# ashispati/ar-vae

Measured on AMD Instinct MI355X. Metric: training images/sec (dSprites beta-VAE+AR, per-GPU batch 512), higher is better.
Workload: dtype f32 (conv MFMAs: scaled 2-term fp16 split, 3 products, fp32-accurate)

## Files before the change

### ar-vae_amd/csrc/common.h

```cpp
#pragma once
#include <hip/hip_runtime.h>
#include <stdint.h>
#include <stdio.h>

#include "../../include/arvae_hip.h"

namespace arvae {

extern thread_local char g_last_error[512];

int fail(int code, const char *fmt, ...);
int check_launch(const char *what);
void prof_gap();
bool profiling_active();

#define ARVAE_LAUNCH(...)                  \
    do {                                   \
        ::arvae::prof_gap();               \
        hipLaunchKernelGGL(__VA_ARGS__);   \
    } while (0)

#define ARVAE_REQUIRE(cond, ...)                                   \
    do {                                                           \
        if (!(cond)) return ::arvae::fail(ARVAE_E_INVALID, __VA_ARGS__); \
    } while (0)

static inline int sample_filter_check(const char *who, const arvae_sample_filter_t *filter, int32_t vocab, int *k_eff, bool *active) {
    ARVAE_REQUIRE(filter != nullptr, "%s: null filter", who);
    ARVAE_REQUIRE(filter->top_k >= 0 && filter->top_k <= vocab, "%s: top_k %d is outside [0, %d] (0 = off)", who, filter->top_k, vocab);
    ARVAE_REQUIRE(filter->top_p > 0.f && filter->top_p <= 1.f, "%s: top_p %f is not in (0, 1] (1 = off)", who,
                  (double)filter->top_p);
    *k_eff = filter->top_k == 0 ? vocab : filter->top_k;
    *active = *k_eff < vocab || filter->top_p < 1.f || filter->allow != nullptr;
    return ARVAE_OK;
}

static inline int note_plan_check(const char *who, const arvae_note_plan_t *plan, int64_t ticks, int32_t vocab) {
    ARVAE_REQUIRE(plan != nullptr, "%s: null plan", who);
    ARVAE_REQUIRE(plan->allow != nullptr, "%s: null plan mask (plan->allow)", who);
    ARVAE_REQUIRE(ticks >= 1 && vocab >= 1, "%s: a plan of %lld ticks and %d notes", who, (long long)ticks, vocab);
// ... 193 lines not shown
```

### ar-vae_amd/csrc/conv32.hip

```cpp
#include "diag.h"
#include "launch.h"
#include "conv32_common.h"
#include "conv32.h"
#include "reduce.h"
#include "midprep.h"
#include "prep32.h"
#include "regloss.h"
#include "down32p.h"
#include "wgrad32r.h"
#include "stamps.h"

#include <type_traits>

namespace arvae {

template <int LO, int STRIDE, int PX = 128>
struct PatchLoader {
    using T = Tile<LO, PX>;
    static constexpr int SZ = STRIDE * LO;
    static constexpr int PR = STRIDE * T::TR + 2, PC = STRIDE * T::TC + 2;
    static constexpr int SLOTS = T::TI * PR * PC * 8;
    static constexpr int ITERS = (SLOTS + 255) / 256;
    float4 r[ITERS];
    unsigned rel[ITERS];
// ... 71 lines not shown
                uint2 hv, lv;
                split2(r[it].x, r[it].y, sc, hv.x, lv.x);
                split2(r[it].z, r[it].w, sc, hv.y, lv.y);
                unsigned *d = buf + pix * PSB2 + q * 2;
                *reinterpret_cast<uint2 *>(d) = hv;
                *reinterpret_cast<uint2 *>(d + 16) = lv;
            }
        }
    }
};

#ifdef ARVAE_STAMPS_CONV32
ARVAE_STAMP_TABLE(conv32, 512, 64, 2)
#define STAMP(slot) do { if (LO == 16 && threadIdx.x == 0) ARVAE_STAMP(g_conv32_stamps, BID, slot); } while (0)
#define STAMP_WAIT() stamp_wait_all()
#define PSTAMP(role, slot) do { if (threadIdx.x == 256 * (role) && BID < 256) ARVAE_STAMP(g_conv32_stamps, BID + 256 * (role), slot); } while (0)
#else
#define STAMP(slot)
#define STAMP_WAIT()
#define PSTAMP(role, slot)
#endif


template <int MODE>
__device__ __forceinline__ unsigned store_group(const f32x16 &acc, int g, float inv, const float4 &b, const float4 &gv, unsigned gbits,
                                                __amdgpu_buffer_rsrc_t rs_out, unsigned off, bool live, float &amax) {
    float v[4] = {fmaf(acc[4 * g], inv, b.x), fmaf(acc[4 * g + 1], inv, b.y), fmaf(acc[4 * g + 2], inv, b.z), fmaf(acc[4 * g + 3], inv, b.w)};
    const float gf[4] = {gv.x, gv.y, gv.z, gv.w};
    unsigned bits = 0;
#pragma unroll
    for (int j = 0; j < 4; ++j) {
        if (MODE == EP_RELU) {
            v[j] = fmaxf(v[j], 0.f);
            bits |= (v[j] > 0.f ? 1u : 0u) << (4 * g + j);
        }
        if (MODE == EP_GATE_F) v[j] = gf[j] > 0.f ? v[j] : 0.f;
        if (MODE == EP_GATE_B) v[j] = ((gbits >> (4 * g + j)) & 1u) ? v[j] : 0.f;
    }
    const float4 o = make_float4(v[0], v[1], v[2], v[3]);
    amax = live ? fmaxf(amax, amax4(o)) : amax;
    buf_store4(o, rs_out, off + g * 32);
    return bits;
}

template <int MODE>
__device__ __forceinline__ void store_pixel(const f32x16 &acc, float inv, const float4 (&b4)[4], __amdgpu_buffer_rsrc_t rs_out,
                                            __amdgpu_buffer_rsrc_t rs_gate, __amdgpu_buffer_rsrc_t rs_bits, bool want_bits,
                                            unsigned off, int half, bool live, float &amax) {
    float4 gv[4];
    unsigned gb = 0;
#pragma unroll
    for (int g = 0; g < 4; ++g) gv[g] = make_float4(0.f, 0.f, 0.f, 0.f);
    if (MODE == EP_GATE_F) {
#pragma unroll
        for (int g = 0; g < 4; ++g) gv[g] = buf_load4(rs_gate, off + g * 32);
    }
    if (MODE == EP_GATE_B) gb = buf_load_u16(rs_bits, bits_off(off, half));
    unsigned bits = 0;
#pragma unroll
    for (int g = 0; g < 4; ++g) bits |= store_group<MODE>(acc, g, inv, b4[g], gv[g], gb, rs_out, off, live, amax);
    if (MODE == EP_RELU && want_bits) buf_store_u16(bits, rs_bits, bits_off(off, half));
}

__device__ __forceinline__ void load_bias4(const float *bias, int half, float4 (&b4)[4]) {
#pragma unroll
    for (int g = 0; g < 4; ++g)
        b4[g] = bias != nullptr ? *reinterpret_cast<const float4 *>(bias + 8 * g + 4 * half) : make_float4(0.f, 0.f, 0.f, 0.f);
}

__global__ __launch_bounds__(256) void conv32_weight_prep_kernel(PrepArgs p) { conv32_prep_block(p, blockIdx.x); }

__global__ __launch_bounds__(256) void prep_all_kernel(PrepArgs p, MidPrepArgs mid, int conv_blocks) {
    prep_all_block(p, mid, conv_blocks, blockIdx.x);
}

__global__ __launch_bounds__(256) void amax_kernel(const float *__restrict__ x, int64_t count4, unsigned *__restrict__ out) {
    __shared__ float wm[4];
    float m = 0.f;
    const int64_t stride = (int64_t)gridDim.x * 256;
    for (int64_t i = (int64_t)blockIdx.x * 256 + threadIdx.x; i < count4; i += 4 * stride) {
        float4 v[4];
#pragma unroll
        for (int u = 0; u < 4; ++u) {
// ... 64 lines not shown
            tile_origin<LO, PX>(tile + NBLK, ni, nr);
            pl.set_tile(ni, nr, tile + NBLK < n_tiles);
            pl.issue_all();
        }
        f32x16 acc;
#pragma unroll
        for (int i = 0; i < 16; ++i) acc[i] = 0.f;
#pragma unroll
        for (int kx = 0; kx < 4; ++kx)
#pragma unroll
            for (int cc = 0; cc < 2; ++cc) {
                const f16x8 ah = lds_x8<f16x8>(ldsw + aoff + kx * PSB2 + cc * 8), al = lds_x8<f16x8>(ldsw + aoff + kx * PSB2 + cc * 8 + 16);
                MFMA_H(acc, w2[kx][cc][1], ah);
                MFMA_H(acc, w2[kx][cc][0], al);
                MFMA_H(acc, w2[kx][cc][0], ah);
            }
#pragma unroll
        for (int reg = 0; reg < 16; ++reg) red[(wave * 16 + reg) * 64 + lane] = acc[reg];
        __syncthreads();
        if (wave == 0) {
#pragma unroll
            for (int reg = 0; reg < 16; ++reg)
                acc[reg] = (acc[reg] + red[(16 + reg) * 64 + lane]) + (red[(32 + reg) * 64 + lane] + red[(48 + reg) * 64 + lane]);
            store_pixel<MODE>(acc, inv, b4, rs_out, rs_gate, rs_bits, want_bits,
                              out_lane + (unsigned)(((img0 * LO + r0) * LO) * PIXB), half, true, amax_run);
        }
    }
    if (wave == 0) amax_publish(ep.amax_out, BID, NBLK, amax_run);
}
template <int LO, int MODE>
__global__ __launch_bounds__(256, 2) void down32s_kernel(const float *__restrict__ hi, Ep32 ep, int n_img, int n_tiles) {
    down32s_body<LO, MODE>(hi, ep, n_img, n_tiles, blockIdx.x, gridDim.x);
}



constexpr int UP_ISSUE_STEPS = 4;
template <int LO, int MODE, int PX = 128>
__device__ __forceinline__ void up32x_body(const float *__restrict__ lo, Ep32 ep, int n_img, int n_tiles, const int BID, const int NBLK) {
    using PL = PatchLoader<LO, 1, PX>;
    constexpr int MT = PX / 32;
    constexpr int HI = 2 * LO, PC = PL::PC, PR = PL::PR, PLANE = PL::PLANE_DW;
    extern __shared__ __attribute__((aligned(16))) float lds[];
    unsigned *ldsw = reinterpret_cast<unsigned *>(lds);
    const int lane = threadIdx.x & 63, wave = __builtin_amdgcn_readfirstlane(threadIdx.x >> 6);
    const int half = lane >> 5, rc = lane & 31;
    const int py = wave >> 1, px = wave & 1;
// ... 79 lines not shown
#pragma unroll
        for (int mt = 0; mt < MT; ++mt)
#pragma unroll
            for (int i = 0; i < 16; ++i) acc[mt][i] = 0.f;
        f16x8 a[2][MT][2];
#pragma unroll
        for (int mt = 0; mt < MT; ++mt)
#pragma unroll
            for (int t = 0; t < 2; ++t) a[0][mt][t] = lds_x8<f16x8>(ldsw + t * PLANE + aoff[mt]);
        static_for<0, 8>([&](auto sc_) __attribute__((always_inline)) {
            constexpr int step = decltype(sc_)::value, ty = step >> 2, tx = (step >> 1) & 1, c = step & 1;
            constexpr int cur = step & 1, nxt = cur ^ 1;
            constexpr int nstep = step + 1, nty = nstep >> 2, ntx = (nstep >> 1) & 1, nc = nstep & 1;
            constexpr int ntoff = -(nty * PC + ntx) * PSB + nc * 8;
            if constexpr (step < UP_ISSUE_STEPS) pl.template issue_step<UP_ISSUE_STEPS, step>();
            __builtin_amdgcn_sched_barrier(0);
            static_for<0, MT>([&](auto mc) __attribute__((always_inline)) {
                constexpr int sub = decltype(mc)::value;
                constexpr int slot = step * MT + sub;
                if constexpr ((slot & 1) == 0) {
                    constexpr int k = slot >> 1, em = k >> 2, eg = k & 3;
                    const unsigned poff = prev_base + orel[em];
                    if (eg == 0) pbits[em] = 0;
                    pbits[em] |= store_group<MODE>(prev[em], eg, inv, b4[eg], gq[k], gqb[em], rs_out, poff, prev_base != OOB, amax_run);
                    if (MODE == EP_RELU && eg == 3)
                        buf_store_u16(pbits[em], rs_bits, (prev_base == OOB || !want_bits) ? OOB : bits_off(poff, half));
                    if (MODE == EP_GATE_F) gq[k] = buf_load4(rs_gate, obase + orel[em] + eg * 32);
                    if constexpr (MODE == EP_GATE_B && k < MT) gqn[k] = buf_load_u16(rs_bits, bits_off(obase + orel[k], half));
                }
                static_for<3 * sub, 3 * sub + 3>([&](auto qc) __attribute__((always_inline)) {
                    constexpr int m = decltype(qc)::value, prod = m / MT, pm = m % MT;
                    constexpr int tw = prod == 0 ? 1 : 0, ta = prod == 1 ? 1 : 0;
                    MFMA_H(acc[pm], w2[ty][tx][c][tw], a[cur][pm][ta]);
                });
                if constexpr (nstep < 8) {
                    static_for<2 * sub, 2 * sub + 2>([&](auto rc_) __attribute__((always_inline)) {
                        constexpr int ri = decltype(rc_)::value, rmt = ri / 2, rt = ri % 2;
                        a[nxt][rmt][rt] = lds_x8<f16x8>(ldsw + rt * PLANE + aoff[rmt] + ntoff);
                    });
                }
                (void)nxt;
            });
            __builtin_amdgcn_sched_barrier(0);
        });
        STAMP(7 + 6 * stamp_t);
#pragma unroll
        for (int mt = 0; mt < MT; ++mt) prev[mt] = acc[mt];
        if (MODE == EP_GATE_B) {
#pragma unroll
            for (int mt = 0; mt < MT; ++mt) gqb[mt] = gqn[mt];
        }
        prev_base = obase;
        __syncthreads();
        pl.commit_split2(ldsw, sc.s);
        __syncthreads();
        STAMP(8 + 6 * stamp_t);
        ++stamp_t;
    }
#pragma unroll
    for (int mt = 0; mt < MT; ++mt) {
        const unsigned poff = prev_base + orel[mt];
        unsigned bits = 0;
#pragma unroll
        for (int g = 0; g < 4; ++g) bits |= store_group<MODE>(prev[mt], g, inv, b4[g], gq[mt * 4 + g], gqb[mt], rs_out, poff, prev_base != OOB, amax_run);
        if (MODE == EP_RELU) buf_store_u16(bits, rs_bits, (prev_base == OOB || !want_bits) ? OOB : bits_off(poff, half));
    }
    amax_publish(ep.amax_out, BID * 4 + wave, NBLK * 4, amax_run);
    STAMP_WAIT();
    STAMP(63);
}
template <int LO, int MODE, int PX = 128>
__global__ __launch_bounds__(256, 1) void up32x_kernel(const float *__restrict__ lo, Ep32 ep, int n_img, int n_tiles) {
    up32x_body<LO, MODE, PX>(lo, ep, n_img, n_tiles, blockIdx.x, gridDim.x);
}

struct C1Wgrad {
    const float *img;
    float *slab;
};
constexpr int C1W_VP = 16, C1W_XP = 16;
constexpr int C1W_WAVE_DW = 2 * 32 * C1W_VP + 2 * 32 * C1W_XP;
constexpr float C1W_SX = 1024.f, C1W_SX_INV = 1.f / 1024.f;

template <int MODE, bool C1W = false>
__device__ __forceinline__ void up32p_body(const float *__restrict__ lo, Ep32 ep, int n_img, int n_tiles, const int BID, const int NBLK,
                                           C1Wgrad c1 = C1Wgrad{nullptr, nullptr}) {
    static_assert(MODE != EP_GATE_F, "up32p_kernel: float gates stay on up32x_kernel");
    static_assert(!C1W || MODE == EP_GATE_B, "the fused first-layer weight gradient takes the sign-bit gated data gradient");
    constexpr int LO = 16, PX = 128, HI = 2 * LO, MT = PX / 32;
    using PL = PatchLoader<LO, 1, PX>;
    constexpr int PR = PL::PR, PC = PL::PC, PLANE = PL::PLANE_DW, SLOTS = PL::SLOTS, ITERS = PL::ITERS;
    constexpr int BUF = 2 * PLANE;
    extern __shared__ __attribute__((aligned(16))) float lds_f[];
    unsigned *lds = reinterpret_cast<unsigned *>(lds_f);
    float4 *hand = reinterpret_cast<float4 *>(lds + 2 * BUF);
    const int lane = threadIdx.x & 63, wave = __builtin_amdgcn_readfirstlane(threadIdx.x >> 6);
    const int half = lane >> 5, rc = lane & 31;
    const int per_wg = (n_tiles + NBLK - 1) / NBLK, t_first = BID * per_wg;
    const int t_end = min(n_tiles, t_first + per_wg);
    const int cls = wave & 3, py = cls >> 1, px = cls & 1;

    if (wave >= 4) {
        PSTAMP(1, 0);
        int pst = 0;
        (void)pst;
        const AmaxLoad al = amax_issue(ep.amax_in);
        unsigned orel[MT];
#pragma unroll
        for (int mt = 0; mt < MT; ++mt) {
            int img, r, c;
            tile_pixel<LO, PX>(mt * 32 + rc, img, r, c);
            orel[mt] = (unsigned)(((img * HI + 2 * r + py) * HI + 2 * c + px) * PIXB + half * 16);
        }
        const int64_t out_bytes = (int64_t)n_img * HI * HI * PIXB;
        const __amdgpu_buffer_rsrc_t rs_out = make_rsrc(ep.out, out_bytes);
        const bool want_bits = MODE == EP_RELU && ep.bits_out != nullptr;
        const __amdgpu_buffer_rsrc_t rs_bits =
            make_rsrc(MODE == EP_GATE_B ? (const void *)ep.gate_bits : want_bits ? (const void *)ep.bits_out : (const void *)ep.out,
                      (int64_t)n_img * HI * HI * 4);
        float4 b4[4];
        load_bias4(ep.bias, half, b4);
        const float inv = amax_scale(al).inv * prep_inv_scale(ep.wprep);
        float amax_run = 0.f;
        auto tile_base = [&](int tile) -> unsigned {
            int img0, r0;
            tile_origin<LO, PX>(tile, img0, r0);
            return tile < t_end ? (unsigned)(((img0 * HI + 2 * r0) * HI) * PIXB) : OOB;
        };
        unsigned gb[MT] = {}, gbn[MT] = {};
        auto request_gates = [&](unsigned base) __attribute__((always_inline)) {
            if (MODE == EP_GATE_B) {
#pragma unroll
                for (int mt = 0; mt < MT; ++mt) gbn[mt] = buf_load_u16(rs_bits, base == OOB ? OOB : bits_off(base + orel[mt], half));
            }
        };
        auto epilogue = [&](unsigned base) __attribute__((always_inline)) {
            const float4 no_gate = make_float4(0.f, 0.f, 0.f, 0.f);
#pragma unroll
            for (int mt = 0; mt < MT; ++mt) {
                f32x16 acc;
#pragma unroll
                for (int g = 0; g < 4; ++g) {
                    const float4 v = hand[((cls * MT + mt) * 4 + g) * 64 + lane];
                    acc[4 * g] = v.x; acc[4 * g + 1] = v.y; acc[4 * g + 2] = v.z; acc[4 * g + 3] = v.w;
                }
                const unsigned poff = base + orel[mt];
                unsigned bits = 0;
#pragma unroll
                for (int g = 0; g < 4; ++g) bits |= store_group<MODE>(acc, g, inv, b4[g], no_gate, gb[mt], rs_out, poff, base != OOB, amax_run);
                if (MODE == EP_RELU) buf_store_u16(bits, rs_bits, (base == OOB || !want_bits) ? OOB : bits_off(poff, half));
            }
        };
        unsigned *c1_v = lds + 2 * BUF + 4 * MT * 4 * 64 * 4 + (wave - 4) * C1W_WAVE_DW;
        unsigned *c1_x = c1_v + 2 * 32 * C1W_VP;
        f32x16 c1_acc, c1_acc2;
#pragma unroll
        for (int i = 0; i < 16; ++i) { c1_acc[i] = 0.f; c1_acc2[i] = 0.f; }
        const __amdgpu_buffer_rsrc_t rs_img = make_rsrc(C1W ? c1.img : ep.out, C1W ? (int64_t)n_img * 4 * HI * HI * 4 : 0);
        int c1_voff[2][2], c1_xoff[2][2];
        const int c1_sw = 2 * ((rc >> 2) & 7);
        {
            const int g16 = lane >> 4, q = (lane & 15) >> 2, pp = lane & 3;
#pragma unroll
            for (int b = 0; b < 2; ++b)
#pragma unroll
                for (int i = 0; i < 2; ++i) {
                    const int P = 16 * b + 8 * (g16 >> 1) + 4 * i + q;
                    const int sw = 2 * ((P >> 2) & 7);
                    c1_voff[b][i] = P * C1W_VP + ((8 * (g16 & 1) + 2 * pp) ^ sw);
                    c1_xoff[b][i] = P * C1W_XP + ((8 * (g16 & 1) + 2 * pp) ^ sw);
                }
            if constexpr (C1W) {
                const int csw = 2 * ((rc >> 2) & 7);
#pragma unroll
                for (int d = 0; d < 4; ++d) {
                    const int col = 8 + 4 * half + d;
// ... 7 lines not shown
            if constexpr (C1W) {
                int img0, r0;
                tile_origin<LO, PX>(tile, img0, r0);
#pragma unroll
                for (int mt = 0; mt < MT; ++mt) {
                    int im, r, c;
                    tile_pixel<LO, PX>(mt * 32 + rc, im, r, c);
                    const int Y = 2 * (r0 + r) + py, X = 2 * c + px;
#pragma unroll
                    for (int e = 0; e < 2; ++e) {
                        const int iy = 2 * Y - 1 + 2 * half + e, ix = X == 0 ? 0 : 2 * X - 1;
                        const bool ok = tile < t_end && (unsigned)iy < (unsigned)(2 * HI);
                        c1_tapn[mt][e] = buf_load4(rs_img, ok ? (unsigned)((((img0 + im) * 2 * HI + iy) * 2 * HI + ix) * 4) : OOB);
                    }
                }
            }
        };
        auto c1_tile = [&](unsigned base) __attribute__((always_inline)) {
            if constexpr (C1W) {
#pragma unroll
                for (int mt = 0; mt < MT; ++mt) {
#pragma unroll
                    for (int g = 0; g < 4; ++g) {
                        const float4 a = hand[((cls * MT + mt) * 4 + g) * 64 + lane];
                        const unsigned bits = base != OOB ? gb[mt] >> (4 * g) : 0u;
                        const float v0 = (bits & 1u) ? a.x : 0.f, v1 = (bits & 2u) ? a.y : 0.f, v2 = (bits & 4u) ? a.z : 0.f, v3 = (bits & 8u) ? a.w : 0.f;
                        uint2 hv, lv;
                        split2(v0, v1, 0x1p-23f, hv.x, lv.x);
                        split2(v2, v3, 0x1p-23f, hv.y, lv.y);
                        const int vd = (4 * g + 2 * half) ^ c1_sw;
                        *reinterpret_cast<uint2 *>(c1_v + rc * C1W_VP + vd) = hv;
                        *reinterpret_cast<uint2 *>(c1_v + 32 * C1W_VP + rc * C1W_VP + vd) = lv;
                    }
                    {
                        int im, r, c;
                        tile_pixel<LO, PX>(mt * 32 + rc, im, r, c);
                        const int X = 2 * c + px;
                        uint4 hx, lx;
                        unsigned *hp = &hx.x, *lp = &lx.x;
#pragma unroll
                        for (int e = 0; e < 2; ++e) {
                            float4 t = c1_tap[mt][e];
                            if (X == 0) t = make_float4(0.f, t.x, t.y, t.z);
                            if (X == HI - 1) t.w = 0.f;
                            split2(t.x, t.y, C1W_SX, hp[2 * e], lp[2 * e]);
                            split2(t.z, t.w, C1W_SX, hp[2 * e + 1], lp[2 * e + 1]);
                        }
// ... 169 lines not shown
                    constexpr int m = decltype(qc)::value, prod = m / MT, pm = m % MT;
                    constexpr int tw = prod == 0 ? 1 : 0, ta = prod == 1 ? 1 : 0;
                    MFMA_H(acc[pm], w2[ty][tx][c][tw], a[cu][pm][ta]);
                });
                if constexpr (nstep < 8) {
                    static_for<2 * sub, 2 * sub + 2>([&](auto rc_) __attribute__((always_inline)) {
                        constexpr int ri = decltype(rc_)::value, rmt = ri / 2, rt = ri % 2;
                        a[nxt][rmt][rt] = lds_x8<f16x8>(ldsw + rt * PLANE + aoff[rmt] + ntoff);
                    });
                }
                (void)nxt;
                __builtin_amdgcn_sched_barrier(0);
            });
        });
        PSTAMP(0, 4 + 6 * cst);
        commit_tile(lds + (cur ^ 1) * BUF);
        PSTAMP(0, 5 + 6 * cst);
        __syncthreads();
        PSTAMP(0, 6 + 6 * cst);
#pragma unroll
        for (int mt = 0; mt < MT; ++mt)
#pragma unroll
            for (int g = 0; g < 4; ++g)
                hand[((wave * MT + mt) * 4 + g) * 64 + lane] = make_float4(acc[mt][4 * g], acc[mt][4 * g + 1], acc[mt][4 * g + 2], acc[mt][4 * g + 3]);
        PSTAMP(0, 7 + 6 * cst);
        __syncthreads();
        PSTAMP(0, 8 + 6 * cst);
        ++cst;
    }
    PSTAMP(0, 63);
    if constexpr (C1W) {
        __syncthreads();
        __syncthreads();
    }
}
template <int MODE>
__global__ __launch_bounds__(512) __attribute__((amdgpu_waves_per_eu(2, 2))) void up32p_kernel(const float *__restrict__ lo, Ep32 ep,
                                                                                               int n_img, int n_tiles) {
    up32p_body<MODE>(lo, ep, n_img, n_tiles, blockIdx.x, gridDim.x);
}

template <int LO, int MODE>
__global__ __launch_bounds__(256, 1) void up32x_reg_kernel(const float *__restrict__ lo, Ep32 ep, int n_img,
                                                            int n_tiles, int grid_up, RegArgs reg, int reg_bx) {
    if ((int)blockIdx.x < grid_up) {
        up32x_body<LO, MODE, 32>(lo, ep, n_img, n_tiles, blockIdx.x, grid_up);
        return;
// ... 82 lines not shown
            set_lo(ni, nr, tile + NBLK < n_tiles);
        }
        static_for<0, KB>([&](auto bc) __attribute__((always_inline)) {
            constexpr int b = decltype(bc)::value;
            f16x8 b2[2];
#pragma unroll
            for (int t = 0; t < 2; ++t) b2[t] = lds_tr_x8<f16x8>(lo_w + t * LPLANE + loff[b][0], lo_w + t * LPLANE + loff[b][1]);
            pl.template issue_step<KB, b>();
            if constexpr (b < 2) lr[b] = buf_load4(rs_lo, lo_base + b * 4096);
#pragma unroll
            for (int kx = 0; kx < 4; ++kx) {
                f16x8 a2[2];
#pragma unroll
                for (int t = 0; t < 2; ++t)
                    a2[t] = lds_tr_x8<f16x8>(ldsw + t * PLANE + hoff[b][0] + kx * WG_PSB_H, ldsw + t * PLANE + hoff[b][1] + kx * WG_PSB_H);
                MFMA_H(acc[kx], a2[1], b2[0]);
                MFMA_H(acc[kx], a2[0], b2[1]);
                MFMA_H(acc[kx], a2[0], b2[0]);
            }
        });
    }

    float *out = slab + (int64_t)BID * WG32_SLAB;
    const float inv = sc_lo.inv * sc_hi.inv;
#pragma unroll
    for (int kx = 0; kx < 4; ++kx)
#pragma unroll
        for (int g = 0; g < 4; ++g)
            *reinterpret_cast<float4 *>(out + ((wave * 4 + kx) * C32 + rc) * C32 + 8 * g + 4 * half) =
                make_float4(acc[kx][4 * g] * inv, acc[kx][4 * g + 1] * inv, acc[kx][4 * g + 2] * inv, acc[kx][4 * g + 3] * inv);
    if (BIAS != 0) {
        __syncthreads();
        *reinterpret_cast<float4 *>(lds + threadIdx.x * 4) = bias4;
        __syncthreads();
        if (threadIdx.x < C32) {
            const int q = threadIdx.x >> 2, e = threadIdx.x & 3;
            float tot = 0.f;
            for (int j = 0; j < 32; ++j) tot += lds[(j * 8 + q) * 4 + e];
            out[16 * C32 * C32 + threadIdx.x] = tot;
        }
    }
}
template <int LO, int BIAS>
__global__ __launch_bounds__(256, 1) void wgrad32x_kernel(const float *__restrict__ lo, const float *__restrict__ hi,
                                                          float *__restrict__ slab, int n_img, int n_tiles, const unsigned *amax_lo,
                                                          const unsigned *amax_hi) {
    wgrad32x_body<LO, BIAS>(lo, hi, slab, n_img, n_tiles, amax_lo, amax_hi, blockIdx.x, gridDim.x);
}

template <int MODE, int BIAS>
__global__ __launch_bounds__(256, 1) void pair4_down_kernel(const float *__restrict__ g_hi, Ep32 ep,
                                                           const float *__restrict__ w_lo, const float *__restrict__ w_hi,
                                                           float *__restrict__ slab, int n_img, int tiles_a, int tiles_b, int grid_a,
// ... 48 lines not shown

bool conv32_fits(const arvae_link_t *l) {
    return l->chi == 32 && l->clo == 32 && l->kh == 4 && l->kw == 4 && l->stride == 2 && l->pad == 1 &&
           l->hh == l->hw && l->lh == l->lw && (l->lh == 16 || l->lh == 8 || l->lh == 4) && l->hi_perm_c == 0 &&
           l->lo_perm_c == 0 && (int64_t)l->n * l->hh * l->hw * PIXB < (1ll << 31) - (1ll << 20);
}

template <int A, int B> struct MaxOf { static constexpr int value = A > B ? A : B; };

constexpr int LDS_DOWN_S = (PatchLoader<4, 2, 32>::BUF2_DW + 4 * 16 * 64) * 4;
static int down_small_grid(int tiles) {
    int g = tiles < 2 * cu_count() ? tiles : 2 * cu_count();
    return g < AMAX_N ? g : AMAX_N;
}

template <int MODE> static void launch_down_small(const Operand &hi, const Ep32 &ep, int n, hipStream_t s) {
    const int tiles = tiles_for<4, 32>(n);
    launch_lds<down32s_kernel<4, MODE>>(dim3(down_small_grid(tiles)), dim3(256), LDS_DOWN_S, s, hi.v, ep, n, tiles);
}
template <int LO, int MODE, int PX>
static void launch_up_px(const Operand &lo, const Ep32 &ep, int n, hipStream_t s) {
    const int tiles = tiles_for<LO, PX>(n), grid = grid_for_tiles(tiles);
    if constexpr (LO == 16 && PX == 128 && MODE != EP_GATE_F) {
        constexpr int LDSP = (2 * 2 * PatchLoader<16, 1, 128>::PLANE_DW) * 4 + 4 * 4 * 4 * 64 * 16;
        launch_lds<up32p_kernel<MODE>>(dim3(grid), dim3(512), LDSP, s, lo.v, ep, n, tiles);
    } else {
        constexpr int LDSX = 2 * PatchLoader<LO, 1, PX>::PLANE_DW * 4;
        launch_lds<up32x_kernel<LO, MODE, PX>>(dim3(grid), dim3(256), LDSX, s, lo.v, ep, n, tiles);
    }
}
template <int LO, int MODE>
static void launch_up_v(const Operand &lo, const Ep32 &ep, int n, hipStream_t s) {
    if (LO == 4 && 2 * tiles_for<LO, 128>(n) <= cu_count()) launch_up_px<4, MODE, 32>(lo, ep, n, s);
    else if (LO == 8 && tiles_for<LO, 128>(n) <= cu_count()) launch_up_px<8, MODE, 32>(lo, ep, n, s);
    else launch_up_px<LO, MODE, 128>(lo, ep, n, s);
}

static int ep_mode(const Ep32 &ep, int relu) {
    return ep.gate_bits != nullptr ? EP_GATE_B : ep.gate != nullptr ? EP_GATE_F : relu ? EP_RELU : EP_PLAIN;
}

template <int LO, int MODE> static void launch_down_p(const float *hi, const Ep32 &ep, int n, hipStream_t s) {
    constexpr int LDS = DownK<LO>::LDS_DW * 4;
    const int tiles = n * DownK<LO>::TILES_PER_IMG;
    launch_lds<down32p_kernel<LO, MODE>>(dim3(grid_for_tiles(tiles)), dim3(512), LDS, s, hi, ep, n, tiles);
}
template <class F> static bool with_ep_mode(int mode, F &&f) { return with_int<EP_GATE_B, EP_GATE_F, EP_RELU, EP_PLAIN>(mode, f); }
// ... 202 lines not shown
                                             const unsigned *amax_g, const unsigned *amax_x, hipStream_t s, int *grid_b_out,
                                             const C1Wgrad *c1 = nullptr, int *grid_a_out = nullptr) {
    const int cus = cu_count() < AMAX_N / 4 ? cu_count() : AMAX_N / 4;
    int grid_a = cus * (c1 != nullptr ? PAIR_SPLIT_C1_PERCENT : PAIR_SPLIT_PERCENT) / 100;
    if (grid_a < 1) grid_a = 1;
    const int tiles_a = up ? l->n * DownK<LO>::TILES_PER_IMG : (LO == 16 ? tiles_for<16, 128>(l->n) : tiles_for<8, 32>(l->n));
    {
        const int run = (tiles_a + grid_a - 1) / grid_a;
        grid_a = (tiles_a + run - 1) / run;
    }
    if (grid_a_out != nullptr) *grid_a_out = grid_a;
    ARVAE_REQUIRE(c1 == nullptr || grid_a <= 256, "pair_up16_wgrad: %d workgroups of the Up half exceed the first layer's 256 weight-gradient slabs", grid_a);
    int total, spw, grid_b;
    stream_geometry(l, cus - grid_a, total, spw, grid_b);
    *grid_b_out = grid_b;
    constexpr int LDS_W = RowStream<LO>::LDS_DW * 4;
    const dim3 grid(grid_a + grid_b);
    if (up) {
        constexpr int LDS = MaxOf<LDS_W, DownK<LO>::LDS_DW * 4>::value;
        launch_lds<pair_down_wgrad_kernel<LO, EP_GATE_B, 2>>(grid, dim3(512), LDS, s, g, ep, l->n, tiles_a, grid_a, x_in, g, slab, total, spw, amax_x, amax_g);
        return check_launch(LO == 16 ? "pair(down32<16> + wgrad32<16>)" : "pair(down32<8> + wgrad32<8>)");
    }
    if constexpr (LO == 16) {
        constexpr int LDS_U = (2 * 2 * PatchLoader<16, 1, 128>::PLANE_DW) * 4 + 4 * 4 * 4 * 64 * 16;
        constexpr int LDS = MaxOf<LDS_W, LDS_U>::value;
        if (c1 != nullptr) {
            constexpr int LDS_C = MaxOf<LDS_W, LDS_U + 4 * C1W_WAVE_DW * 4>::value;
            launch_lds<pair_up16_wgrad_kernel<EP_GATE_B, 1, true>>(grid, dim3(512), LDS_C, s, g, ep, l->n, tiles_a, grid_a, g, x_in, slab, total, spw,
                                                                   amax_g, amax_x, *c1);
            return check_launch("pair(up32<16> + wgrad32<16> + wgrad_c1)");
        }
        launch_lds<pair_up16_wgrad_kernel<EP_GATE_B, 1>>(grid, dim3(512), LDS, s, g, ep, l->n, tiles_a, grid_a, g, x_in, slab, total, spw, amax_g,
                                                         amax_x, C1Wgrad{nullptr, nullptr});
        return check_launch("pair(up32<16> + wgrad32<16>)");
    } else {
        constexpr int LDS = MaxOf<LDS_W, 2 * PatchLoader<8, 1, 32>::PLANE_DW * 4>::value;
        launch_lds<pair_up8_wgrad_kernel<EP_GATE_B, 1>>(grid, dim3(512), LDS, s, g, ep, l->n, tiles_a, grid_a, g, x_in, slab, total, spw, amax_g, amax_x);
        return check_launch("pair(up32<8> + wgrad32<8>)");
    }
}

bool conv32_pair_c1_fits(const arvae_link_t *l, bool up, const uint16_t *gate_bits) {
    return !up && l->lh == 16 && gate_bits != nullptr;
}
int conv32_pair(const arvae_link_t *l, bool up, const float *g, const float *x_in, const float *gate, const uint16_t *gate_bits,
                float *d_in, const float *wprep, float *dwt, float *dbias, float *slab, hipStream_t s, SlabJob *job,
                const unsigned *amax_g, const unsigned *amax_x, unsigned *amax_out, const float *c1_img, float *c1_slab, SlabJob *c1_job) {
// ... 40 lines not shown
```

### ar-vae_amd/csrc/conv32_common.h

```cpp
#pragma once
#include "common.h"
#include "splitmath.h"
#include "amax.h"

#include <type_traits>

namespace arvae {

constexpr int C32 = 32;
constexpr int PSB2 = 36;
constexpr int PSB = 20;
constexpr int WGRAD_PSB_H = 24, WGRAD_PSB_L = 16;
constexpr int PIXB = C32 * 4;
constexpr unsigned OOB = 0x7fffffffu;

template <int LO, int PX = 128> struct Tile {
    static constexpr int ROWS = PX / LO;
    static constexpr int TI = ROWS > LO ? ROWS / LO : 1, TR = ROWS > LO ? LO : ROWS, TC = LO;
};

template <int LO, int PX = 128> __device__ __forceinline__ constexpr void tile_pixel(int p, int &img, int &r, int &c) {
    using T = Tile<LO, PX>;
    c = p % T::TC;
    r = (p / T::TC) % T::TR;
// ... 11 lines not shown
        static_for<I + 1, N>(f);
    }
}

enum { EP_PLAIN = 0, EP_RELU = 1, EP_GATE_F = 2, EP_GATE_B = 3 };
struct Ep32 {
    const float *bias;
    const float *gate;
    const uint16_t *gate_bits;
    uint16_t *bits_out;
    float *out;
    const uint4 *wprep;
    const unsigned *amax_in;
    unsigned *amax_out;
};

__device__ __forceinline__ __amdgpu_buffer_rsrc_t make_rsrc(const void *p, int64_t bytes) {
    return __builtin_amdgcn_make_buffer_rsrc(const_cast<void *>(p), 0, (int)bytes, 0x00020000);
}
__device__ __forceinline__ float4 buf_load4(__amdgpu_buffer_rsrc_t r, unsigned off) {
    const f32x4 v = __builtin_bit_cast(f32x4, __builtin_amdgcn_raw_buffer_load_b128(r, (int)off, 0, 0));
    return make_float4(v.x, v.y, v.z, v.w);
}
__device__ __forceinline__ void buf_store4(float4 v, __amdgpu_buffer_rsrc_t r, unsigned off) {
    f32x4 q;
    q.x = v.x; q.y = v.y; q.z = v.z; q.w = v.w;
    __builtin_amdgcn_raw_buffer_store_b128(__builtin_bit_cast(i32x4, q), r, (int)off, 0, 0);
}

__device__ __forceinline__ unsigned buf_load_u16(__amdgpu_buffer_rsrc_t r, unsigned off) {
    return (unsigned)(unsigned short)__builtin_amdgcn_raw_buffer_load_b16(r, (int)off, 0, 0);
}
__device__ __forceinline__ void buf_store_u16(unsigned v, __amdgpu_buffer_rsrc_t r, unsigned off) {
    __builtin_amdgcn_raw_buffer_store_b16((unsigned short)v, r, (int)off, 0, 0);
}

constexpr int PREP_DOWN_SLOTS = 32, PREP_UP_SLOTS = 16;
constexpr int PREP_DOWN_UINT4 = 2 * PREP_DOWN_SLOTS * 64, PREP_UP_UINT4 = 4 * PREP_UP_SLOTS * 64;
constexpr int PREP_FLOATS = (PREP_DOWN_UINT4 + PREP_UP_UINT4 + 1) * 4;
__device__ __forceinline__ float prep_inv_scale(const uint4 *wprep) {
    return __builtin_bit_cast(float, wprep[PREP_DOWN_UINT4 + PREP_UP_UINT4].x);
}

__device__ __forceinline__ unsigned bits_off(unsigned out_off, int half) { return (out_off >> 7) * 4 + half * 2; }

}
```

### ar-vae_amd/csrc/down32p.h

```cpp
#pragma once
#include "common.h"
#include "conv32_common.h"
#include "stamps.h"

namespace arvae {

#ifdef ARVAE_STAMPS_D32K
ARVAE_STAMP_TABLE(d32k, 64, 64, 1)
#define DSTAMP(role, slot) do { if (LO == 16 && threadIdx.x == 256 * (role) && BID < 32) ARVAE_STAMP(g_d32k_stamps, BID + 32 * (role), slot); } while (0)
#else
#define DSTAMP(role, slot)
#endif

template <int LO> struct DownK {
    using T = Tile<LO, 64>;
    static constexpr int HW = 2 * LO;
    static constexpr int PR = 2 * T::TR + 2;
    static constexpr int PIX = PR * HW;
    static constexpr int BUF = (PIX + 1) * PSB2;
    static constexpr int SLOTS = (PIX * 8 + 255) / 256;
    static constexpr int XCH = 4 * 3 * 2 * 64 * 4;
    static constexpr int LDS_DW = 2 * BUF + XCH;
    static constexpr int TILES_PER_IMG = LO / T::TR;
};

template <int LO, int MODE, int CHAIN = 0>
__device__ __forceinline__ void down32p_body(const float *__restrict__ hi, Ep32 ep, int n_img, int n_tiles, const int BID, const int NBLK,
                                             float *chain_max = nullptr) {
    using K = DownK<LO>;
    constexpr int HW = K::HW, PIX = K::PIX, SLOTS = K::SLOTS, HI = 2 * LO;
    extern __shared__ __attribute__((aligned(16))) unsigned ldsd[];
    unsigned *xch = ldsd + 2 * K::BUF;
    const int lane = threadIdx.x & 63, wave = __builtin_amdgcn_readfirstlane(threadIdx.x >> 6);
    const int per_wg = (n_tiles + NBLK - 1) / NBLK, t_first = BID * per_wg;
    const int t_end = min(n_tiles, t_first + per_wg);
    using S0 = std::integral_constant<int, 0>;
    using S1 = std::integral_constant<int, 1>;
    auto chain_scale = [&]() __attribute__((always_inline)) -> Pow2 {
        const float m = fmaxf(fmaxf(chain_max[0], chain_max[1]), fmaxf(chain_max[2], chain_max[3]));
        return pow2_for((unsigned)__builtin_amdgcn_readfirstlane(__builtin_bit_cast(int, m)));
    };

    if (wave >= 4) {
        DSTAMP(1, 0);
        int pst = 0;
        (void)pst;
        const int pt = threadIdx.x - 256;
        const __amdgpu_buffer_rsrc_t rs_hi = make_rsrc(hi, (int64_t)n_img * HI * HI * PIXB);
        int q = pt & 7, pix0 = pt >> 3;
        float4 lv[2][SLOTS];
        float sc_in = 1.f;
        AmaxLoad al{};
        if constexpr (CHAIN != 2) al = amax_issue(ep.amax_in);
// ... 131 lines not shown
            for (int k = 0; k < 3; ++k) part[e][k] = xq_own[(k * 2 + e) * 64];
    };
    auto epi_item = [&](auto ic) __attribute__((always_inline)) {
        constexpr int i = decltype(ic)::value;
        if constexpr (i < 8) {
            constexpr int e = i / 4, k = i % 4;
            if constexpr (k < 3) {
                const float4 p = part[e][k];
                own[e].x += p.x; own[e].y += p.y; own[e].z += p.z; own[e].w += p.w;
            } else {
                float o4[4] = {fmaf(own[e].x, inv, b4[e].x), fmaf(own[e].y, inv, b4[e].y), fmaf(own[e].z, inv, b4[e].z), fmaf(own[e].w, inv, b4[e].w)};
                const float gf[4] = {gq_prev[e].x, gq_prev[e].y, gq_prev[e].z, gq_prev[e].w};
#pragma unroll
                for (int j = 0; j < 4; ++j) {
                    if (MODE == EP_RELU) {
                        o4[j] = fmaxf(o4[j], 0.f);
                        bits_acc |= (o4[j] > 0.f ? 1u : 0u) << (4 * e + j);
                    }
                    if (MODE == EP_GATE_F) o4[j] = gf[j] > 0.f ? o4[j] : 0.f;
                    if (MODE == EP_GATE_B) o4[j] = ((gb_prev >> (8 * og + 4 * e + j)) & 1u) ? o4[j] : 0.f;
                }
                const float4 ov = make_float4(o4[0], o4[1], o4[2], o4[3]);
                amax_run = obase_prev != OOB ? fmaxf(amax_run, amax4(ov)) : amax_run;
                buf_store4(ov, rs_out, obase_prev + e * 32);
            }
        } else if constexpr (i == 8) {
            if (MODE == EP_RELU)
                __builtin_amdgcn_raw_buffer_store_b8((unsigned char)bits_acc, rs_bits,
                                                     (int)((obase_prev == OOB || !want_bits) ? OOB : bits_off(obase_prev, half) + og), 0, 0);
            bits_acc = 0;
        }
    };
    auto do_tile = [&](int tile, int cur) __attribute__((always_inline)) {
        DSTAMP(0, 4 + 5 * cst);
        const unsigned *xb = ldsd + cur * K::BUF;
        f32x16 acc[2], accb[2];
#pragma unroll
        for (int mt = 0; mt < 2; ++mt)
#pragma unroll
            for (int i = 0; i < 16; ++i) { acc[mt][i] = 0.f; accb[mt][i] = 0.f; }
        f16x8 x2[2][2][2];
#pragma unroll
        for (int mt = 0; mt < 2; ++mt)
#pragma unroll
            for (int t = 0; t < 2; ++t)
                x2[0][mt][t] = lds_x8<f16x8>(xb + xoff[mt][0] + t * 16);
        load_parts();
// ... 93 lines not shown
```

### ar-vae_amd/csrc/wgrad32r.h

```cpp
#pragma once
#include "common.h"
#include "conv32_common.h"
#include "reduce.h"
#include "stamps.h"

namespace arvae {

template <int LO> struct RowStream {
    static constexpr int HW = 2 * LO;
    static constexpr int RB = HW * PIXB;
    static constexpr int HN = 16384 / RB;
    static constexpr int TR = 32 / LO;
    static constexpr int RING = 3 * HN;
    static constexpr int PCOLS = HW + 2;
    static constexpr int HP = WGRAD_PSB_H, LP = WGRAD_PSB_L;
    static constexpr int HPLANE = RING * PCOLS * HP;
    static constexpr int LPLANE = 32 * LP, LBUF = 2 * LPLANE;
    static constexpr int LDS_DW = 2 * HPLANE + 2 * LBUF;
    static constexpr int PRO = 2 * RB / 4096;
    static constexpr int STEPS_PER_IMG = LO * LO / 32;
};

#ifdef ARVAE_STAMPS_WGR
ARVAE_STAMP_TABLE(wgr, 512, 64, 2)
// ... 177 lines not shown
              __builtin_amdgcn_sched_group_barrier(0x008, 1, 0); __builtin_amdgcn_sched_group_barrier(0x100, 4, 0); } \
          _Pragma("unroll") for (int g_ = 0; g_ < 4; ++g_) {                                                      \
              __builtin_amdgcn_sched_group_barrier(0x008, 1, 0); __builtin_amdgcn_sched_group_barrier(0x100, 2, 0); } }
        for (int k = k0; k < k1; ++k) {
            __builtin_amdgcn_sched_barrier(0);
            mask_b(std::integral_constant<int, 0>{}, k);
            read_block(std::integral_constant<int, 1>{});
            mfma_block(std::integral_constant<int, 0>{});
            ARVAE_WGR_INTERLEAVE
            __builtin_amdgcn_sched_barrier(0);
            WGR_STAMP(0, 2 + 2 * (k - k0));
            __syncthreads();
            WGR_STAMP(0, 3 + 2 * (k - k0));
            set_step(k + 1);
            mask_b(std::integral_constant<int, 1>{}, k);
            __builtin_amdgcn_sched_barrier(0);
            read_block(std::integral_constant<int, 0>{});
            mfma_block(std::integral_constant<int, 1>{});
            ARVAE_WGR_INTERLEAVE
            __builtin_amdgcn_sched_barrier(0);
        }
#undef ARVAE_WGR_INTERLEAVE
        WGR_STAMP(0, 62);
#pragma unroll
        for (int kx = 0; kx < 4; ++kx)
#pragma unroll
            for (int g = 0; g < 4; ++g)
                *reinterpret_cast<float4 *>(out + ((wave * 4 + kx) * C32 + rc) * C32 + 8 * g + 4 * half) =
                    make_float4(acc[kx][4 * g] * inv, acc[kx][4 * g + 1] * inv, acc[kx][4 * g + 2] * inv, acc[kx][4 * g + 3] * inv);
        WGR_STAMP(0, 63);
    }
    if (BIAS != 0) {
        __syncthreads();
        if (threadIdx.x < C32) {
            const float *red = reinterpret_cast<const float *>(ring);
            const int qq = threadIdx.x >> 2, e = threadIdx.x & 3;
            float tot = 0.f;
            for (int j = 0; j < 32; ++j) tot += red[(j * 8 + qq) * 4 + e];
            out[16 * C32 * C32 + threadIdx.x] = tot;
        }
    }
}

template <int LO, int BIAS>
__global__ __launch_bounds__(512, 2) void wgrad32r_kernel(const float *__restrict__ lo, const float *__restrict__ hi,
                                                          float *__restrict__ slab, int n_img, int total_steps, int steps_per_wg,
                                                          const unsigned *amax_lo, const unsigned *amax_hi) {
    wgrad32r_body<LO, BIAS>(lo, hi, slab, n_img, total_steps, steps_per_wg, amax_lo, amax_hi, blockIdx.x);
}

}
```

Baseline: 1.366 million.

## Add store cache policies and coalesce conv epilogue and wgrad slab stores

Adds a store-policy layer that passes a cache-policy bit (value 16) to buffer stores. The 32x32 activation outputs and the wgrad slab use this non-default policy, while the other stores stay plain. The up32p handoff buffer in LDS is re-laid out (padded) so the store waves write contiguous 16-byte channel chunks per pixel, with the relu and gate bits exchanged through shuffles. The wgrad32r slab write is staged through a padded per-wave LDS tile so each wave issues fully coalesced 128-bit stores. The aim is to cut partial-line write traffic and keep streaming outputs from polluting cache, at the cost of extra LDS traffic, shuffles and wave barriers.

```diff
diff --git a/ar-vae_amd/csrc/common.h b/ar-vae_amd/csrc/common.h
--- a/ar-vae_amd/csrc/common.h
+++ b/ar-vae_amd/csrc/common.h
@@ -4,6 +4,7 @@
 #include <stdio.h>
 
 #include "../../include/arvae_hip.h"
+#include "storepolicy.h"
 
 namespace arvae {
 
@@ -16,6 +17,7 @@
 
 #define ARVAE_LAUNCH(...)                  \
     do {                                   \
+        ::arvae::store_policy_sync();      \
         ::arvae::prof_gap();               \
         hipLaunchKernelGGL(__VA_ARGS__);   \
     } while (0)
diff --git a/ar-vae_amd/csrc/conv32.hip b/ar-vae_amd/csrc/conv32.hip
--- a/ar-vae_amd/csrc/conv32.hip
+++ b/ar-vae_amd/csrc/conv32.hip
@@ -117,7 +117,7 @@
 #endif
 
 
-template <int MODE>
+template <int MODE, int POL>
 __device__ __forceinline__ unsigned store_group(const f32x16 &acc, int g, float inv, const float4 &b, const float4 &gv, unsigned gbits,
                                                 __amdgpu_buffer_rsrc_t rs_out, unsigned off, bool live, float &amax) {
     float v[4] = {fmaf(acc[4 * g], inv, b.x), fmaf(acc[4 * g + 1], inv, b.y), fmaf(acc[4 * g + 2], inv, b.z), fmaf(acc[4 * g + 3], inv, b.w)};
@@ -134,11 +134,11 @@
     }
     const float4 o = make_float4(v[0], v[1], v[2], v[3]);
     amax = live ? fmaxf(amax, amax4(o)) : amax;
-    buf_store4(o, rs_out, off + g * 32);
+    buf_store4<POL>(o, rs_out, off + g * 32);
     return bits;
 }
 
-template <int MODE>
+template <int MODE, int POL>
 __device__ __forceinline__ void store_pixel(const f32x16 &acc, float inv, const float4 (&b4)[4], __amdgpu_buffer_rsrc_t rs_out,
                                             __amdgpu_buffer_rsrc_t rs_gate, __amdgpu_buffer_rsrc_t rs_bits, bool want_bits,
                                             unsigned off, int half, bool live, float &amax) {
@@ -153,7 +153,7 @@
     if (MODE == EP_GATE_B) gb = buf_load_u16(rs_bits, bits_off(off, half));
     unsigned bits = 0;
 #pragma unroll
-    for (int g = 0; g < 4; ++g) bits |= store_group<MODE>(acc, g, inv, b4[g], gv[g], gb, rs_out, off, live, amax);
+    for (int g = 0; g < 4; ++g) bits |= store_group<MODE, POL>(acc, g, inv, b4[g], gv[g], gb, rs_out, off, live, amax);
     if (MODE == EP_RELU && want_bits) buf_store_u16(bits, rs_bits, bits_off(off, half));
 }
 
@@ -264,7 +264,7 @@
 #pragma unroll
             for (int reg = 0; reg < 16; ++reg)
                 acc[reg] = (acc[reg] + red[(16 + reg) * 64 + lane]) + (red[(32 + reg) * 64 + lane] + red[(48 + reg) * 64 + lane]);
-            store_pixel<MODE>(acc, inv, b4, rs_out, rs_gate, rs_bits, want_bits,
+            store_pixel<MODE, st_map32<LO>()>(acc, inv, b4, rs_out, rs_gate, rs_bits, want_bits,
                               out_lane + (unsigned)(((img0 * LO + r0) * LO) * PIXB), half, true, amax_run);
         }
     }
@@ -390,7 +390,7 @@
                     constexpr int k = slot >> 1, em = k >> 2, eg = k & 3;
                     const unsigned poff = prev_base + orel[em];
                     if (eg == 0) pbits[em] = 0;
-                    pbits[em] |= store_group<MODE>(prev[em], eg, inv, b4[eg], gq[k], gqb[em], rs_out, poff, prev_base != OOB, amax_run);
+                    pbits[em] |= store_group<MODE, st_map32<HI>()>(prev[em], eg, inv, b4[eg], gq[k], gqb[em], rs_out, poff, prev_base != OOB, amax_run);
                     if (MODE == EP_RELU && eg == 3)
                         buf_store_u16(pbits[em], rs_bits, (prev_base == OOB || !want_bits) ? OOB : bits_off(poff, half));
                     if (MODE == EP_GATE_F) gq[k] = buf_load4(rs_gate, obase + orel[em] + eg * 32);
@@ -430,7 +430,7 @@
         const unsigned poff = prev_base + orel[mt];
         unsigned bits = 0;
 #pragma unroll
-        for (int g = 0; g < 4; ++g) bits |= store_group<MODE>(prev[mt], g, inv, b4[g], gq[mt * 4 + g], gqb[mt], rs_out, poff, prev_base != OOB, amax_run);
+        for (int g = 0; g < 4; ++g) bits |= store_group<MODE, st_map32<HI>()>(prev[mt], g, inv, b4[g], gq[mt * 4 + g], gqb[mt], rs_out, poff, prev_base != OOB, amax_run);
         if (MODE == EP_RELU) buf_store_u16(bits, rs_bits, (prev_base == OOB || !want_bits) ? OOB : bits_off(poff, half));
     }
     amax_publish(ep.amax_out, BID * 4 + wave, NBLK * 4, amax_run);
@@ -449,6 +449,7 @@
 constexpr int C1W_VP = 16, C1W_XP = 16;
 constexpr int C1W_WAVE_DW = 2 * 32 * C1W_VP + 2 * 32 * C1W_XP;
 constexpr float C1W_SX = 1024.f, C1W_SX_INV = 1.f / 1024.f;
+constexpr int HAND_H = 33, HAND_G = 66, HAND_MT = 4 * HAND_G, UP32P_HAND_F4 = 4 * 4 * HAND_MT;
 
 template <int MODE, bool C1W = false>
 __device__ __forceinline__ void up32p_body(const float *__restrict__ lo, Ep32 ep, int n_img, int n_tiles, const int BID, const int NBLK,
@@ -473,21 +474,17 @@
         int pst = 0;
         (void)pst;
         const AmaxLoad al = amax_issue(ep.amax_in);
-        unsigned orel[MT];
-#pragma unroll
-        for (int mt = 0; mt < MT; ++mt) {
-            int img, r, c;
-            tile_pixel<LO, PX>(mt * 32 + rc, img, r, c);
-            orel[mt] = (unsigned)(((img * HI + 2 * r + py) * HI + 2 * c + px) * PIXB + half * 16);
-        }
+        const int p8 = lane >> 3, ch = lane & 7, cg = ch >> 1, chh = ch & 1;
+        const unsigned orel_lane = (unsigned)((py * HI + 2 * p8 + px) * PIXB + ch * 16);
+        auto orel_of = [&](int mt, int i) -> unsigned { return orel_lane + (unsigned)(((2 * (2 * mt + (i >> 1))) * HI + 16 * (i & 1)) * PIXB); };
+        static_assert(Tile<LO, PX>::TC == 16 && Tile<LO, PX>::TI == 1, "the store waves' pixel walk is written for 8-row tiles of one image");
         const int64_t out_bytes = (int64_t)n_img * HI * HI * PIXB;
         const __amdgpu_buffer_rsrc_t rs_out = make_rsrc(ep.out, out_bytes);
         const bool want_bits = MODE == EP_RELU && ep.bits_out != nullptr;
         const __amdgpu_buffer_rsrc_t rs_bits =
             make_rsrc(MODE == EP_GATE_B ? (const void *)ep.gate_bits : want_bits ? (const void *)ep.bits_out : (const void *)ep.out,
                       (int64_t)n_img * HI * HI * 4);
-        float4 b4[4];
-        load_bias4(ep.bias, half, b4);
+        const float4 bq = ep.bias != nullptr ? *reinterpret_cast<const float4 *>(ep.bias + 4 * ch) : make_float4(0.f, 0.f, 0.f, 0.f);
         const float inv = amax_scale(al).inv * prep_inv_scale(ep.wprep);
         float amax_run = 0.f;
         auto tile_base = [&](int tile) -> unsigned {
@@ -499,27 +496,45 @@
         auto request_gates = [&](unsigned base) __attribute__((always_inline)) {
             if (MODE == EP_GATE_B) {
 #pragma unroll
-                for (int mt = 0; mt < MT; ++mt) gbn[mt] = buf_load_u16(rs_bits, base == OOB ? OOB : bits_off(base + orel[mt], half));
+                for (int mt = 0; mt < MT; ++mt) {
+                    int img, r, c;
+                    tile_pixel<LO, PX>(mt * 32 + rc, img, r, c);
+                    const unsigned acc_px = (unsigned)(((2 * r + py) * HI + 2 * c + px) * PIXB);
+                    gbn[mt] = buf_load_u16(rs_bits, base == OOB ? OOB : C1W ? bits_off(base + acc_px, half) : bits_off(base + orel_of(mt, cg), chh));
+                }
             }
         };
         auto epilogue = [&](unsigned base) __attribute__((always_inline)) {
-            const float4 no_gate = make_float4(0.f, 0.f, 0.f, 0.f);
 #pragma unroll
             for (int mt = 0; mt < MT; ++mt) {
-                f32x16 acc;
-#pragma unroll
-                for (int g = 0; g < 4; ++g) {
-                    const float4 v = hand[((cls * MT + mt) * 4 + g) * 64 + lane];
-                    acc[4 * g] = v.x; acc[4 * g + 1] = v.y; acc[4 * g + 2] = v.z; acc[4 * g + 3] = v.w;
+                unsigned mine = 0;
+#pragma unroll
+                for (int i = 0; i < 4; ++i) {
+                    const float4 a = hand[(cls * MT + mt) * HAND_MT + cg * HAND_G + chh * HAND_H + 8 * i + p8];
+                    float v[4] = {fmaf(a.x, inv, bq.x), fmaf(a.y, inv, bq.y), fmaf(a.z, inv, bq.z), fmaf(a.w, inv, bq.w)};
+                    unsigned gate = 0, bits = 0;
+                    if (MODE == EP_GATE_B) gate = (unsigned)__shfl((int)gb[mt], (lane & ~6) | (i << 1)) >> (4 * cg);
+#pragma unroll
+                    for (int j = 0; j < 4; ++j) {
+                        if (MODE == EP_RELU) {
+                            v[j] = fmaxf(v[j], 0.f);
+                            bits |= (v[j] > 0.f ? 1u : 0u) << (4 * cg + j);
+                        }
+                        if (MODE == EP_GATE_B) v[j] = ((gate >> j) & 1u) ? v[j] : 0.f;
+                    }
+                    const float4 o = make_float4(v[0], v[1], v[2], v[3]);
+                    amax_run = base != OOB ? fmaxf(amax_run, amax4(o)) : amax_run;
+                    buf_store4<st_map32<HI>()>(o, rs_out, base + orel_of(mt, i));
+                    if (MODE == EP_RELU) {
+                        bits |= (unsigned)__shfl_xor((int)bits, 2);
+                        bits |= (unsigned)__shfl_xor((int)bits, 4);
+                        mine = cg == i ? bits : mine;
+                    }
                 }
-                const unsigned poff = base + orel[mt];
-                unsigned bits = 0;
-#pragma unroll
-                for (int g = 0; g < 4; ++g) bits |= store_group<MODE>(acc, g, inv, b4[g], no_gate, gb[mt], rs_out, poff, base != OOB, amax_run);
-                if (MODE == EP_RELU) buf_store_u16(bits, rs_bits, (base == OOB || !want_bits) ? OOB : bits_off(poff, half));
+                if (MODE == EP_RELU) buf_store_u16(mine, rs_bits, (base == OOB || !want_bits) ? OOB : bits_off(base + orel_of(mt, cg), chh));
             }
         };
-        unsigned *c1_v = lds + 2 * BUF + 4 * MT * 4 * 64 * 4 + (wave - 4) * C1W_WAVE_DW;
+        unsigned *c1_v = lds + 2 * BUF + UP32P_HAND_F4 * 4 + (wave - 4) * C1W_WAVE_DW;
         unsigned *c1_x = c1_v + 2 * 32 * C1W_VP;
         f32x16 c1_acc, c1_acc2;
 #pragma unroll
@@ -573,7 +588,7 @@
                 for (int mt = 0; mt < MT; ++mt) {
 #pragma unroll
                     for (int g = 0; g < 4; ++g) {
-                        const float4 a = hand[((cls * MT + mt) * 4 + g) * 64 + lane];
+                        const float4 a = hand[(cls * MT + mt) * HAND_MT + g * HAND_G + half * HAND_H + rc];
                         const unsigned bits = base != OOB ? gb[mt] >> (4 * g) : 0u;
                         const float v0 = (bits & 1u) ? a.x : 0.f, v1 = (bits & 2u) ? a.y : 0.f, v2 = (bits & 4u) ? a.z : 0.f, v3 = (bits & 8u) ? a.w : 0.f;
                         uint2 hv, lv;
@@ -789,7 +804,7 @@
         for (int mt = 0; mt < MT; ++mt)
 #pragma unroll
             for (int g = 0; g < 4; ++g)
-                hand[((wave * MT + mt) * 4 + g) * 64 + lane] = make_float4(acc[mt][4 * g], acc[mt][4 * g + 1], acc[mt][4 * g + 2], acc[mt][4 * g + 3]);
+                hand[(wave * MT + mt) * HAND_MT + g * HAND_G + half * HAND_H + rc] = make_float4(acc[mt][4 * g], acc[mt][4 * g + 1], acc[mt][4 * g + 2], acc[mt][4 * g + 3]);
         PSTAMP(0, 7 + 6 * cst);
         __syncthreads();
         PSTAMP(0, 8 + 6 * cst);
@@ -918,13 +933,14 @@
     }
 
     float *out = slab + (int64_t)BID * WG32_SLAB;
+    const __amdgpu_buffer_rsrc_t rs_slab = make_rsrc(out, (int64_t)WG32_SLAB * 4);
     const float inv = sc_lo.inv * sc_hi.inv;
 #pragma unroll
     for (int kx = 0; kx < 4; ++kx)
 #pragma unroll
         for (int g = 0; g < 4; ++g)
-            *reinterpret_cast<float4 *>(out + ((wave * 4 + kx) * C32 + rc) * C32 + 8 * g + 4 * half) =
-                make_float4(acc[kx][4 * g] * inv, acc[kx][4 * g + 1] * inv, acc[kx][4 * g + 2] * inv, acc[kx][4 * g + 3] * inv);
+            buf_store4<ST_SLAB4>(make_float4(acc[kx][4 * g] * inv, acc[kx][4 * g + 1] * inv, acc[kx][4 * g + 2] * inv, acc[kx][4 * g + 3] * inv),
+                                rs_slab, (unsigned)((((wave * 4 + kx) * C32 + rc) * C32 + 8 * g + 4 * half) * 4));
     if (BIAS != 0) {
         __syncthreads();
         *reinterpret_cast<float4 *>(lds + threadIdx.x * 4) = bias4;
@@ -1019,7 +1035,7 @@
 static void launch_up_px(const Operand &lo, const Ep32 &ep, int n, hipStream_t s) {
     const int tiles = tiles_for<LO, PX>(n), grid = grid_for_tiles(tiles);
     if constexpr (LO == 16 && PX == 128 && MODE != EP_GATE_F) {
-        constexpr int LDSP = (2 * 2 * PatchLoader<16, 1, 128>::PLANE_DW) * 4 + 4 * 4 * 4 * 64 * 16;
+        constexpr int LDSP = (2 * 2 * PatchLoader<16, 1, 128>::PLANE_DW) * 4 + UP32P_HAND_F4 * 16;
         launch_lds<up32p_kernel<MODE>>(dim3(grid), dim3(512), LDSP, s, lo.v, ep, n, tiles);
     } else {
         constexpr int LDSX = 2 * PatchLoader<LO, 1, PX>::PLANE_DW * 4;
@@ -1268,7 +1284,7 @@
         return check_launch(LO == 16 ? "pair(down32<16> + wgrad32<16>)" : "pair(down32<8> + wgrad32<8>)");
     }
     if constexpr (LO == 16) {
-        constexpr int LDS_U = (2 * 2 * PatchLoader<16, 1, 128>::PLANE_DW) * 4 + 4 * 4 * 4 * 64 * 16;
+        constexpr int LDS_U = (2 * 2 * PatchLoader<16, 1, 128>::PLANE_DW) * 4 + UP32P_HAND_F4 * 16;
         constexpr int LDS = MaxOf<LDS_W, LDS_U>::value;
         if (c1 != nullptr) {
             constexpr int LDS_C = MaxOf<LDS_W, LDS_U + 4 * C1W_WAVE_DW * 4>::value;
diff --git a/ar-vae_amd/csrc/conv32_common.h b/ar-vae_amd/csrc/conv32_common.h
--- a/ar-vae_amd/csrc/conv32_common.h
+++ b/ar-vae_amd/csrc/conv32_common.h
@@ -57,10 +57,10 @@
     const f32x4 v = __builtin_bit_cast(f32x4, __builtin_amdgcn_raw_buffer_load_b128(r, (int)off, 0, 0));
     return make_float4(v.x, v.y, v.z, v.w);
 }
-__device__ __forceinline__ void buf_store4(float4 v, __amdgpu_buffer_rsrc_t r, unsigned off) {
+template <int POL = ST_PLAIN> __device__ __forceinline__ void buf_store4(float4 v, __amdgpu_buffer_rsrc_t r, unsigned off) {
     f32x4 q;
     q.x = v.x; q.y = v.y; q.z = v.z; q.w = v.w;
-    __builtin_amdgcn_raw_buffer_store_b128(__builtin_bit_cast(i32x4, q), r, (int)off, 0, 0);
+    buf_store_b128<POL>(__builtin_bit_cast(st_i32x4, q), r, (int)off);
 }
 
 __device__ __forceinline__ unsigned buf_load_u16(__amdgpu_buffer_rsrc_t r, unsigned off) {
diff --git a/ar-vae_amd/csrc/down32p.h b/ar-vae_amd/csrc/down32p.h
--- a/ar-vae_amd/csrc/down32p.h
+++ b/ar-vae_amd/csrc/down32p.h
@@ -29,6 +29,7 @@
                                              float *chain_max = nullptr) {
     using K = DownK<LO>;
     constexpr int HW = K::HW, PIX = K::PIX, SLOTS = K::SLOTS, HI = 2 * LO;
+    constexpr int POL = CHAIN == 1 ? ST_CHAIN_A2 : st_map32<LO>();
     extern __shared__ __attribute__((aligned(16))) unsigned ldsd[];
     unsigned *xch = ldsd + 2 * K::BUF;
     const int lane = threadIdx.x & 63, wave = __builtin_amdgcn_readfirstlane(threadIdx.x >> 6);
@@ -206,7 +207,7 @@
                 }
                 const float4 ov = make_float4(o4[0], o4[1], o4[2], o4[3]);
                 amax_run = obase_prev != OOB ? fmaxf(amax_run, amax4(ov)) : amax_run;
-                buf_store4(ov, rs_out, obase_prev + e * 32);
+                buf_store4<POL>(ov, rs_out, obase_prev + e * 32);
             }
         } else if constexpr (i == 8) {
             if (MODE == EP_RELU)
diff --git a/ar-vae_amd/csrc/storepolicy.h b/ar-vae_amd/csrc/storepolicy.h
--- /dev/null
+++ b/ar-vae_amd/csrc/storepolicy.h
@@ -0,0 +1,48 @@
+#pragma once
+#include <hip/hip_runtime.h>
+
+#include "diag.h"
+
+namespace arvae {
+
+constexpr int ST_PLAIN = 0;
+constexpr int ST_WT = 16;
+
+constexpr int ST_SLAB = ST_WT;
+constexpr int ST_SLAB4 = ST_PLAIN;
+constexpr int ST_ACT32 = ST_WT;
+constexpr int ST_ACT16 = ST_PLAIN;
+constexpr int ST_SMALL = ST_PLAIN;
+constexpr int ST_CHAIN_A2 = ST_PLAIN;
+
+template <int SIDE> constexpr int st_map32() { return SIDE >= 32 ? ST_ACT32 : SIDE == 16 ? ST_ACT16 : ST_SMALL; }
+
+#ifdef ARVAE_DIAG
+static __device__ int g_plain_stores;
+static void store_policy_sync() {
+    static const bool done = [] {
+        if (diag_env("ARVAE_PLAIN_STORES") != nullptr) {
+            const int one = 1;
+            (void)hipMemcpyToSymbol(HIP_SYMBOL(g_plain_stores), &one, sizeof(one));
+        }
+        return true;
+    }();
+    (void)done;
+}
+#else
+inline void store_policy_sync() {}
+#endif
+
+typedef int st_i32x4 __attribute__((ext_vector_type(4)));
+
+template <int POL> __device__ __forceinline__ void buf_store_b128(st_i32x4 q, __amdgpu_buffer_rsrc_t r, int off) {
+#ifdef ARVAE_DIAG
+    if (POL != ST_PLAIN && g_plain_stores != 0) {
+        __builtin_amdgcn_raw_buffer_store_b128(q, r, off, 0, ST_PLAIN);
+        return;
+    }
+#endif
+    __builtin_amdgcn_raw_buffer_store_b128(q, r, off, 0, POL);
+}
+
+}
diff --git a/ar-vae_amd/csrc/wgrad32r.h b/ar-vae_amd/csrc/wgrad32r.h
--- a/ar-vae_amd/csrc/wgrad32r.h
+++ b/ar-vae_amd/csrc/wgrad32r.h
@@ -223,12 +223,27 @@
         }
 #undef ARVAE_WGR_INTERLEAVE
         WGR_STAMP(0, 62);
-#pragma unroll
-        for (int kx = 0; kx < 4; ++kx)
-#pragma unroll
-            for (int g = 0; g < 4; ++g)
-                *reinterpret_cast<float4 *>(out + ((wave * 4 + kx) * C32 + rc) * C32 + 8 * g + 4 * half) =
-                    make_float4(acc[kx][4 * g] * inv, acc[kx][4 * g + 1] * inv, acc[kx][4 * g + 2] * inv, acc[kx][4 * g + 3] * inv);
+        const __amdgpu_buffer_rsrc_t rs_slab = make_rsrc(out, (int64_t)SLAB_C32_FLOATS * 4);
+        {
+            constexpr int TP = 36;
+            float *tile = reinterpret_cast<float *>(ring) + 1024 + wave * (C32 * TP);
+            static_assert(1024 + 4 * C32 * TP <= RS::LDS_DW, "the slab tiles fit the ring");
+#pragma unroll
+            for (int kx = 0; kx < 4; ++kx) {
+#pragma unroll
+                for (int g = 0; g < 4; ++g)
+                    *reinterpret_cast<float4 *>(tile + rc * TP + 8 * g + 4 * half) =
+                        make_float4(acc[kx][4 * g] * inv, acc[kx][4 * g + 1] * inv, acc[kx][4 * g + 2] * inv, acc[kx][4 * g + 3] * inv);
+                __builtin_amdgcn_fence(__ATOMIC_RELEASE, "wavefront");
+                __builtin_amdgcn_wave_barrier();
+#pragma unroll
+                for (int i = 0; i < 4; ++i)
+                    buf_store4<ST_SLAB>(*reinterpret_cast<const float4 *>(tile + (8 * i + (lane >> 3)) * TP + 4 * (lane & 7)), rs_slab,
+                                        (unsigned)(((wave * 4 + kx) * C32 * C32) * 4 + (64 * i + lane) * 16));
+                __builtin_amdgcn_fence(__ATOMIC_RELEASE, "wavefront");
+                __builtin_amdgcn_wave_barrier();
+            }
+        }
         WGR_STAMP(0, 63);
     }
     if (BIAS != 0) {
```

After: 1.378 million (median of 6 runs). About the same (+0.8%).
